# Jarvis73/PEMP

Hardware: AMD Instinct MI355X
Metric: episodes/sec (PEMP stage-1 eval step, PASCAL-5i-shaped 1-shot, ResNet-50) (higher is better)
Workload: dtype f32

## Files before the change

### include/pemp_hip.h

```cpp
#ifndef PEMP_HIP_H
#define PEMP_HIP_H

#include <stddef.h>
#include <stdint.h>

#ifdef __cplusplus
extern "C" {
#endif

#define PEMP_ABI_VERSION 2

#define PEMP_CONV_RELU 1u
#define PEMP_CONV_SHIFT_PER_IMAGE 2u
#define PEMP_CONV_STEM4 4u
#define PEMP_CONV_POOL3S2 8u

typedef struct pemp_conv_desc {
    int32_t N, H, W;
    int32_t Cin, ldx;
    int32_t Ho, Wo;
    int32_t Cout, ldy;
    int32_t KH, KW;
    int32_t stride, pad, dil;
    int32_t ldr;
    int32_t Kpad;
    uint32_t flags;
    int32_t tile;
} pemp_conv_desc;

const char* pemp_last_error(void);
// ... 245 lines not shown
```

### pemp_amd/_lib.py

```python
import ctypes as C
import os

import torch

_HERE = os.path.dirname(os.path.abspath(__file__))
LIB_PATH = os.environ.get("PEMP_HIP_LIB", os.path.join(_HERE, "libpemp_hip.so"))

c_fp = C.c_void_p
c_int = C.c_int
c_size = C.c_size_t


class ConvDesc(C.Structure):
    _fields_ = [(n, C.c_int32) for n in
                ("N", "H", "W", "Cin", "ldx", "Ho", "Wo", "Cout", "ldy", "KH", "KW",
                 "stride", "pad", "dil", "ldr", "Kpad")] + [("flags", C.c_uint32), ("tile", C.c_int32)]


class SampleDesc(C.Structure):
    _fields_ = [("img_off", C.c_int64), ("msk_off", C.c_int64), ("img_out", C.c_int64), ("msk_out", C.c_int64)] + \
               [(n, C.c_int32) for n in ("hs", "ws", "sh", "sw", "oy", "ox", "flip", "jitter_order")] + \
               [("jitter", C.c_float * 3), ("mask_mode", C.c_int32), ("ksx", C.c_int32), ("ksy", C.c_int32),
                ("ws_off", C.c_int64)]


CONV_RELU = 1
CONV_SHIFT_PER_IMAGE = 2
CONV_STEM4 = 4
CONV_POOL3S2 = 8

SYMBOLS = {
    "pemp_last_error": (C.c_char_p, []),
    "pemp_abi_version": (c_int, []),
    "pemp_conv2d_hybrid_rows": (c_int, [C.POINTER(ConvDesc)]),
    "pemp_conv2d_tile_shape": (c_int, [c_int, C.POINTER(c_int), C.POINTER(c_int)]),
    "pemp_conv2d_nhwc_f32": (c_int, [C.POINTER(ConvDesc), c_fp, c_fp, c_fp, c_fp, c_fp, c_fp, c_fp]),
    "pemp_conv2d_padv_splitk_nhwc_f32": (c_int, [C.POINTER(ConvDesc), c_fp, c_fp, c_fp, c_fp, c_fp, c_fp, c_fp, c_fp, c_size, c_fp]),
    "pemp_conv2d_padv_nhwc_f32": (c_int, [C.POINTER(ConvDesc), c_fp, c_fp, c_fp, c_fp, c_fp, c_fp, c_fp, c_fp]),
    "pemp_conv2d_group_nhwc_f32": (c_int, [c_int, C.POINTER(ConvDesc)] + [C.POINTER(c_fp)] * 7 + [c_fp]),
    "pemp_conv2d_bf16_nhwc": (c_int, [C.POINTER(ConvDesc), c_fp, c_fp, c_fp, c_fp, c_fp, c_fp, c_fp, c_int, c_fp]),
    "pemp_pack_split3_bf16": (c_int, [c_fp, c_fp, c_int, c_int, c_fp]),
    "pemp_convert_f32_bf16": (c_int, [c_fp, c_fp, C.c_longlong, c_fp]),
    "pemp_convert_bf16_f32": (c_int, [c_fp, c_fp, C.c_longlong, c_fp]),
    "pemp_conv2d_dropblock_nhwc_f32": (c_int, [C.POINTER(ConvDesc), c_fp, c_fp, c_fp, c_fp, c_fp, c_fp, c_fp, c_fp, c_fp, c_size, c_fp]),
# ... 129 lines not shown
```

### pemp_amd/csrc/conv_common.h

```cpp
#pragma once
#include "common.h"

namespace pemp {

typedef __attribute__((ext_vector_type(16))) float f32x16;
typedef __attribute__((ext_vector_type(4))) float v4f;
typedef __attribute__((ext_vector_type(8))) __bf16 bf16x8;
typedef __attribute__((ext_vector_type(2))) unsigned int u32x2;

#define PEMP_CONV_BF16_IO 0x100u

__device__ __forceinline__ v4f load_quad(const float* base, size_t off, unsigned bf16) {
    if (!bf16) return *(const v4f*)(base + off);
    const u32x2 r = *(const u32x2*)((const unsigned short*)base + off);
    return v4f{__builtin_bit_cast(float, r.x << 16), __builtin_bit_cast(float, r.x & 0xFFFF0000u),
               __builtin_bit_cast(float, r.y << 16), __builtin_bit_cast(float, r.y & 0xFFFF0000u)};
}

__device__ __forceinline__ unsigned int bf16_bits(float f) {
    const unsigned int u = __builtin_bit_cast(unsigned int, f);
    if ((u & 0x7FFFFFFFu) > 0x7F800000u) return (u >> 16) | 0x40u;
    return (u + 0x7FFFu + ((u >> 16) & 1u)) >> 16;
}

// ... 32 lines not shown
    float* stats;
    const uint32_t* bmask;
    const float* bz;
    const float* bmean;
    const float* binvstd;
    int ldbz;
    const float* rowmask;
    const int* rowcnt;
    float* sk_ws;
    int* sk_cnt;
    int sk_full, sk_S;
    int N, H, W, Cin, ldx, Ho, Wo, Cout, ldy, KH, KW, stride, pad, dil, ldr, Kpad;
    unsigned flags;
    int M, HoWo, cin_steps, nk, ntaps;
    int bm_first = 0;
};

constexpr int CONV_GROUP_MAX = 4;
struct ConvGroupArgs {
    ConvArgs a[CONV_GROUP_MAX];
    int first[CONV_GROUP_MAX + 1];
    int nblk[CONV_GROUP_MAX];
    int n;
};

__device__ __forceinline__ int xcd_tile_order(int bid, int nblk) {
    const int x = bid & 7, idx = bid >> 3;
    const int q = nblk >> 3, rem = nblk & 7;
    return (x < rem ? x * (q + 1) : rem * (q + 1) + (x - rem) * q) + idx;
}
// ... 192 lines not shown
```

### pemp_amd/csrc/conv_dma2.hip

```cpp
#include "conv_tiles.h"

#ifndef PEMP_SK_ACQUIRE
#define PEMP_SK_ACQUIRE 1
#endif

namespace pemp {

typedef __attribute__((address_space(3))) void* lptr_t;

template <int BM, int BN, int WGM, int NW, bool PADV, int EPI = 0, bool SK = false, bool BF16 = false, bool DB = false, bool R16 = false,
          bool S3 = false>
__device__ __forceinline__ void conv_dma2_body(const ConvArgs& a, const int bid, const int nblk) {
#if defined(__HIP_DEVICE_COMPILE__)
    constexpr int WGN = NW / WGM;
    constexpr int RPI = NW * 8;
    constexpr int WM = BM / WGM, WN = BN / WGN;
    static_assert(!R16 || (WM == 16 && WN % 16 == 0 && EPI == 0 && !SK && !BF16 && !DB), "R16: 16-row wave tiles, plain epilogue only");
    static_assert(!S3 || (EPI == 0 && !BF16 && !DB && !R16), "S3: plain epilogue, fp32 operands");
    constexpr int TM = R16 ? 1 : WM / 32, TN = R16 ? WN / 16 : WN / 32;
    constexpr int BQ = S3 ? 12 : 8;
    static_assert(!S3 || (BN * BQ) % (NW * 64) == 0, "S3: whole B DMA rounds");
    constexpr int AL = BM / RPI, BL = S3 ? BN * BQ / (NW * 64) : BN / RPI;
    constexpr int NMF = S3 ? 6 * TM * TN : R16 ? 2 * TN : TM * TN * (BF16 ? 1 : 4), NDS = S3 ? 2 * TM + 3 * TN : R16 ? 1 + TN : TM + TN,
                  NDMA = AL + BL;
// ... 27 lines not shown
    } else {
        tile_id = xcd_tile_order(bid, nblk);
    }
    const int bm = a.bm_first + tile_id / ntn;
    const int bn = tile_id % ntn;
    const int m0 = bm * BM, n0 = bn * BN;

    const int p = tid & 7;
    const int r = tid >> 3;
    const int sq = p ^ ((r >> 1) & 7);

    const int bias_pix = a.pad * a.W + a.pad;
    const __amdgpu_buffer_rsrc_t rx =
        __builtin_amdgcn_make_buffer_rsrc((void*)(a.x - (ptrdiff_t)bias_pix * a.ldx), 0, 0x80000000u, 0x00020000);
    const __amdgpu_buffer_rsrc_t rw = __builtin_amdgcn_make_buffer_rsrc((void*)a.w, 0, 0x80000000u, 0x00020000);

    const unsigned padv_off = PADV ? (unsigned)((const char*)a.padv - (const char*)(a.x - (ptrdiff_t)bias_pix * a.ldx)) + sq * 16 : 0x80000000u;
    unsigned a_voff[AL], a_inv[AL], b_voff[BL];
#pragma unroll
    for (int i = 0; i < AL; ++i) {
        const int m = m0 + r + RPI * i;
        const bool ok = m < a.M;
        const int mm = ok ? m : 0;
        const int img = mm / a.HoWo;
        const int rem = mm - img * a.HoWo;
        const int ho = rem / a.Wo;
        const int wo = rem - ho * a.Wo;
        const int hi0 = ho * a.stride - a.pad;
        const int wi0 = wo * a.stride - a.pad;
        a_voff[i] = (unsigned)(((img * a.H + hi0) * a.W + wi0 + bias_pix) * a.ldx + sq * 4) * 4u;
// ... 32 lines not shown
            kw_i = __builtin_amdgcn_readfirstlane(tap0 - kh0 * a.KW);
        }
    }
    const int tapw = a.dil * a.ldx * 4, taph = a.dil * a.W * a.ldx * 4;

#define PEMP_DMA2(buf_)                                                                                           \
    do {                                                                                                          \
        v4f* Ad_ = As + (buf_) * BM * 8 + wave * 64;                                                              \
        v4f* Bd_ = Bs + (buf_) * BN * BQ + wave * 64;                                                             \
        const int sa_ = kh_i * taph + kw_i * tapw + cb * 128;                                                     \
        const int sb_ = (tap * a.Cin + cb * 32) * (S3 ? 6 : 4);                                                   \
        const int sh_ = 31 - tap;                                                                                 \
        const unsigned oob_ = PADV ? padv_off - (unsigned)(kh_i * taph + kw_i * tapw) : 0x80000000u;              \
        _Pragma("unroll") for (int i = 0; i < AL; ++i) {                                                          \
            const unsigned vo_ = ((int)(a_inv[i] << sh_) < 0) ? oob_ : a_voff[i];                                 \
            __builtin_amdgcn_raw_ptr_buffer_load_lds(rx, (lptr_t)(Ad_ + i * RPI * 8), 16, vo_, sa_, 0, 0);        \
        }                                                                                                         \
        _Pragma("unroll") for (int i = 0; i < BL; ++i)                                                            \
            __builtin_amdgcn_raw_ptr_buffer_load_lds(rw, (lptr_t)(Bd_ + i * RPI * 8), 16, b_voff[i], sb_, 0, 0);  \
    } while (0)

    int multi, s_kw, s_ntaps;
    asm volatile("s_nop 0\n\tv_readfirstlane_b32 %0, %3\n\tv_readfirstlane_b32 %1, %4\n\tv_readfirstlane_b32 %2, %5\n\ts_nop 4"
                 : "=s"(multi), "=s"(s_kw), "=s"(s_ntaps)
                 : "v"(a.ntaps > 1 ? 1 : 0), "v"(a.KW), "v"(a.ntaps));
#define PEMP_ADVANCE2()                                                                                           \
    do {                                                                                                          \
        int wt_;                                                                                                  \
        asm volatile(                                                                                             \
            "s_add_u32 %0, %0, %5\n\t"                                      \
            "s_add_u32 %2, %2, %5\n\t"                                      \
            "s_cmp_eq_u32 %2, %6\n\t"                                       \
            "s_cselect_b32 %2, 0, %2\n\t"                                   \
            "s_addc_u32 %1, %1, 0\n\t"                                      \
            "s_xor_b32 %4, %5, 1\n\t"                                       \
            "s_cmp_eq_u32 %0, %7\n\t"                                       \
            "s_cselect_b32 %4, 1, %4\n\t"                                                                          \
            "s_cmp_lg_u32 %4, 0\n\t"                                                                               \
            "s_cselect_b32 %0, 0, %0\n\t"                             \
            "s_cselect_b32 %1, 0, %1\n\t"                                                                          \
            "s_cselect_b32 %2, 0, %2\n\t"                                                                          \
            "s_addc_u32 %3, %3, 0"                                                                                \
            : "+s"(tap), "+s"(kh_i), "+s"(kw_i), "+s"(cb), "=&s"(wt_)                                             \
            : "s"(multi), "s"(s_kw), "s"(s_ntaps)                                                    \
            : "scc");                                                                                             \
    } while (0)

    f32x16 acc[R16 ? 1 : TM][R16 ? 1 : TN];
#pragma unroll
    for (int mi = 0; mi < (R16 ? 1 : TM); ++mi)
#pragma unroll
        for (int ni = 0; ni < (R16 ? 1 : TN); ++ni)
#pragma unroll
            for (int e = 0; e < 16; ++e) acc[mi][ni][e] = 0.f;
    v4f acc16[R16 ? TN : 1];
#pragma unroll
    for (int ni = 0; ni < (R16 ? TN : 1); ++ni) acc16[ni] = v4f{0.f, 0.f, 0.f, 0.f};

    PEMP_DMA2(0);
    if (nkl > 1) {
        PEMP_ADVANCE2();
// ... 117 lines not shown
        if (DMA_) {                         \
            _Pragma("unroll") for (int k_ = 0; k_ < NMF; ++k_) {                                                  \
                __builtin_amdgcn_sched_group_barrier(0x008, 1, 0);                                                \
                _Pragma("unroll") for (int q_ = 0; q_ < PER; ++q_) {                                              \
                    const int it_ = k_ * PER + q_;                                                                \
                    if (it_ < NDS) __builtin_amdgcn_sched_group_barrier(0x100, 1, 0);                             \
                    else if (it_ < NDS + NDMA) __builtin_amdgcn_sched_group_barrier(0x020, 1, 0);                 \
                }                                                                                                 \
            }                                                                                                     \
        }                                                                                                         \
        __builtin_amdgcn_sched_barrier(0);                                                                        \
    } while (0)

    int kt = 0;
    PEMP_READ(0, 0, 0);
    for (; kt + 2 < nkl; ++kt) {
        const int buf = kt & 1;
        PEMP_STEP(buf, true, true);
    }
    if (kt + 1 < nkl) {
        const int buf = kt & 1;
        PEMP_STEP(buf, false, true);
        ++kt;
    }
    constexpr bool PRE = !R16 && TM * TN <= 2;
    v4f rpre[PRE ? TM * TN * 4 : 1];
#pragma unroll
    for (int i = 0; i < (PRE ? TM * TN * 4 : 1); ++i) rpre[i] = v4f{0.f, 0.f, 0.f, 0.f};
    if constexpr (PRE) {
        if (a.res) {
            const int rr_ = lane >> 3, c4_ = (lane & 7) * 4;
#pragma unroll
            for (int mi = 0; mi < TM; ++mi)
#pragma unroll
// ... 150 lines not shown
                        o.y = fmaxf(o.y, 0.f);
                        o.z = fmaxf(o.z, 0.f);
                        o.w = fmaxf(o.w, 0.f);
                    }
                    store_quad(a.y, (size_t)m * a.ldy + n, o, a.flags & PEMP_CONV_BF16_IO);
                }
            }
            asm volatile("s_waitcnt lgkmcnt(0)" ::: "memory");
        }
    }
}

template <int BM, int BN, int WGM, int NW, bool PADV>
__device__ __forceinline__ void conv_dma2_s3p_body(const ConvArgs& a) {
#if defined(__HIP_DEVICE_COMPILE__)
    constexpr bool S3 = true, R16 = false, BF16 = false;
    constexpr int WGN = NW / WGM;
    constexpr int RPI = NW * 8;
    constexpr int WM = BM / WGM, WN = BN / WGN;
    constexpr int TM = WM / 32, TN = WN / 32;
    constexpr int BQ = 12;
    static_assert((BN * BQ) % (NW * 64) == 0, "S3: whole B DMA rounds");
    constexpr int AL = BM / RPI, BL = BN * BQ / (NW * 64);
    constexpr int NMF = 6 * TM * TN, NDS = 2 * TM + 3 * TN, NDMA = AL + BL;
    constexpr int PER = (NDS + NDMA + NMF - 1) / NMF;
    constexpr int NST = TM * TN * 4;
    static_assert(NDMA + NST <= 63, "vmcnt range");
    static_assert(NW <= BM / 32 + 3 * BN / 64, "one 4 KB transpose patch per wave inside ONE stage buffer");

    extern __shared__ __attribute__((aligned(16))) v4f smem[];
    v4f* As = smem;
// ... 12 lines not shown
    const int q8 = T >> 3, r8 = T & 7;
    const int t_first = xcd < r8 ? xcd * (q8 + 1) : r8 * (q8 + 1) + (xcd - r8) * q8;
    const int t_cnt = q8 + (xcd < r8 ? 1 : 0);
    const int gx = ((int)gridDim.x - xcd + 7) >> 3;
    if (idx >= t_cnt) return;
    int j = idx;
    int m0 = (a.bm_first + (t_first + j) / ntn) * BM, n0 = ((t_first + j) % ntn) * BN;

    const int p = tid & 7;
    const int r = tid >> 3;
    const int sq = p ^ ((r >> 1) & 7);
    const int bias_pix = a.pad * a.W + a.pad;
    const __amdgpu_buffer_rsrc_t rx =
        __builtin_amdgcn_make_buffer_rsrc((void*)(a.x - (ptrdiff_t)bias_pix * a.ldx), 0, 0x80000000u, 0x00020000);
    const __amdgpu_buffer_rsrc_t rw = __builtin_amdgcn_make_buffer_rsrc((void*)a.w, 0, 0x80000000u, 0x00020000);
    const unsigned padv_off = PADV ? (unsigned)((const char*)a.padv - (const char*)(a.x - (ptrdiff_t)bias_pix * a.ldx)) + sq * 16 : 0x80000000u;
    unsigned a_voff[AL], a_inv[AL], b_voff[BL];
    auto offsets = [&](const int m0_, const int n0_) {
#pragma unroll
        for (int i = 0; i < AL; ++i) {
            const int m = m0_ + r + RPI * i;
            const bool ok = m < a.M;
            const int mm = ok ? m : 0;
            const int img = mm / a.HoWo;
            const int rem = mm - img * a.HoWo;
            const int ho = rem / a.Wo;
            const int wo = rem - ho * a.Wo;
            const int hi0 = ho * a.stride - a.pad;
            const int wi0 = wo * a.stride - a.pad;
            a_voff[i] = (unsigned)(((img * a.H + hi0) * a.W + wi0 + bias_pix) * a.ldx + sq * 4) * 4u;
// ... 52 lines not shown
    int pb = 0;
    for (;;) {
        f32x16 acc[TM][TN];
#pragma unroll
        for (int mi = 0; mi < TM; ++mi)
#pragma unroll
            for (int ni = 0; ni < TN; ++ni)
#pragma unroll
                for (int e = 0; e < 16; ++e) acc[mi][ni][e] = 0.f;
        const int jn = j + gx;
        const bool more = jn < t_cnt;
        const int m0n = more ? (a.bm_first + (t_first + jn) / ntn) * BM : m0, n0n = more ? ((t_first + jn) % ntn) * BN : n0;

        int kt = 0;
        PEMP_READ(0, pb, 0);
        for (; kt + 2 < nkl; ++kt) {
            const int buf = (kt + pb) & 1;
            PEMP_STEP(buf, true, true);
        }
        if (more) {
            offsets(m0n, n0n);
        } else {
#pragma unroll
            for (int i = 0; i < AL; ++i) {
                a_voff[i] = 0x80000000u;
                a_inv[i] = 0u;
            }
#pragma unroll
            for (int i = 0; i < BL; ++i) b_voff[i] = 0x80000000u;
        }
        tap = 0;
        cb = 0;
        kh_i = 0;
        kw_i = 0;
        if (kt + 1 < nkl) {
            const int buf = (kt + pb) & 1;
            PEMP_STEP_X(buf, true, true, false, true);
            ++kt;
        }
        const int bl = (kt + pb) & 1;
        v4f rres[TM * TN * 4], scv[TN], shv[TN];
        auto epi_loads = [&]() {
            const bool per_img = a.flags & PEMP_CONV_SHIFT_PER_IMAGE;
#pragma unroll
            for (int ni = 0; ni < TN; ++ni) {
                const int n = n0 + wn0 + ni * 32 + c4_;
                scv[ni] = a.scale ? *(const v4f*)(a.scale + n) : v4f{1.f, 1.f, 1.f, 1.f};
                shv[ni] = (a.shift && !per_img) ? *(const v4f*)(a.shift + n) : v4f{0.f, 0.f, 0.f, 0.f};
            }
// ... 39 lines not shown
        m0 = m0n;
        n0 = n0n;
        pb = pbn;
    }
#endif
}

template <int BM, int BN, int WGM, int NW, bool PADV>
__global__ __launch_bounds__(NW * 64) __attribute__((amdgpu_waves_per_eu(BM == 64 ? 4 : 2))) void conv_dma2_s3p_kernel(ConvArgs a) {
    conv_dma2_s3p_body<BM, BN, WGM, NW, PADV>(a);
}
#undef PEMP_STEP_X
#undef PEMP_STEP
#undef PEMP_DMA2
#undef PEMP_ADVANCE2
#undef PEMP_READ
#undef PEMP_MMA

template <int BM, int BN, int WGM, int NW, bool PADV, bool R16 = false, bool S3 = false>
__global__ __launch_bounds__(NW * 64) void conv_dma2_group_kernel(ConvGroupArgs g) {
    int which = 0;
#pragma unroll
    for (int i = 1; i < CONV_GROUP_MAX; ++i) which += (i < g.n && (int)blockIdx.x >= g.first[i]) ? 1 : 0;
    const int bid = (int)blockIdx.x - g.first[which];
    if (bid >= g.nblk[which]) return;
    conv_dma2_body<BM, BN, WGM, NW, PADV, 0, false, false, false, R16, S3>(g.a[which], bid, g.nblk[which]);
}


template <class T, bool PADV, int EPI = 0, bool SK = false, bool BF16 = false, bool DB = false, bool R16 = false, bool S3 = false>
// ... 124 lines not shown
    if (grid < 0) return -1;
    return with_tile<FamSplitK>(shape, [&](auto t) {
        using T = decltype(t);
        return launch_with_lds(dma2_fp32_kernel<T, true>(a), grid, T::NW * 64, tile_lds<T>(), st, a, "conv_dma2/splitk");
    });
}

static int split3_check(bool shape_ok, int shape, const ConvArgs& a) {
    if (shape_ok && !a.stats && !a.rowmask && !(a.flags & PEMP_CONV_BF16_IO)) return 0;
    set_error("conv split3: tile %d / epilogue outside the family", shape);
    return -1;
}

int launch_conv_dma2_split3(int shape, ConvArgs a, void* ws, size_t ws_bytes, bool split, hipStream_t st) {
    if (split3_check(in_family<FamSplit3>(shape), shape, a)) return -1;
    const SplitKPlan p = split ? conv_dma2_splitk_plan(shape, a) : SplitKPlan{0, 0, 1, 0};
    const int sk_grid = p.pieces >= 2 ? bind_splitk(a, p, ws, ws_bytes) : 0;
    if (sk_grid < 0) return -1;
    return with_tile<FamSplit3>(shape, [&](auto t) {
        using T = decltype(t);
        auto kern = sk_grid ? (a.padv ? dma2_kernel<T, true, 0, true, false, false, false, true> : dma2_kernel<T, false, 0, true, false, false, false, true>)
                            : (a.padv ? dma2_kernel<T, true, 0, false, false, false, false, true> : dma2_kernel<T, false, 0, false, false, false, false, true>);
        return launch_with_lds(kern, sk_grid ? sk_grid : tile_grid<T>(a), T::NW * 64, tile_lds_s3<T>(), st, a,
                               sk_grid ? "conv_dma2/split3/splitk" : "conv_dma2/split3");
    });
}

template <class T>
static int launch_dma2_s3p(const ConvArgs& a, hipStream_t st) {
    constexpr size_t lds = tile_lds_s3<T>();
// ... 87 lines not shown
```

### pemp_amd/csrc/conv_igemm.hip

```cpp
#include "conv_tiles.h"

namespace pemp {


template <int BM, int BN, int WGM, bool STEM>
__global__ __launch_bounds__(256) void conv_igemm_kernel(ConvArgs a) {
    constexpr int WGN = 4 / WGM;
    constexpr int WM = BM / WGM, WN = BN / WGN;
    constexpr int TM = WM / 32, TN = WN / 32;
    constexpr int AL = BM / 32, BL = BN / 32;
    static_assert(TM >= 1 && TN >= 1, "wave tile");

    extern __shared__ __attribute__((aligned(16))) v4f smem[];
    v4f* As = smem;
    v4f* Bs = smem + 2 * 8 * BM;

    const int tid = threadIdx.x;
    const int lane = tid & 63;
    const int wave = tid >> 6;
    const int wm0 = (wave / WGN) * WM;
    const int wn0 = (wave % WGN) * WN;
    const int lr = lane & 31, lh = lane >> 5;

    const int ntn = a.Cout / BN;
// ... 202 lines not shown

extern "C" int pemp_conv2d_splitk_nhwc_f32(const pemp_conv_desc* d, const float* x, const float* w, float* y,
                                           const float* scale, const float* shift, const float* residual, void* ws,
                                           size_t ws_bytes, void* stream) {
    return conv2d_impl(d, x, w, y, scale, shift, residual, nullptr, ws, ws_bytes, stream);
}

extern "C" int pemp_conv2d_padv_splitk_nhwc_f32(const pemp_conv_desc* d, const float* x, const float* w, float* y,
                                                const float* scale, const float* shift, const float* residual,
                                                const float* pad_value, void* ws, size_t ws_bytes, void* stream) {
    PEMP_REQUIRE(pad_value, "conv2d_padv_splitk: pad_value is null");
    return conv2d_impl(d, x, w, y, scale, shift, residual, pad_value, ws, ws_bytes, stream);
}

static int conv_fill(const pemp_conv_desc* d, const float* x, const float* w, float* y, const float* scale, const float* shift,
                     const float* residual, const float* pad_value, ConvArgs& a, bool any_taps = false, bool pooled = false) {
    PEMP_REQUIRE(d && x && w && y, "conv2d: null pointer");
    PEMP_REQUIRE(pooled || !(d->flags & PEMP_CONV_POOL3S2), "conv2d: PEMP_CONV_POOL3S2 belongs to pemp_conv2d_nhwc_f32 (no grouped / dropblock / statistics / bf16 form)");
    PEMP_REQUIRE(!pad_value || (!(d->flags & PEMP_CONV_STEM4) && (any_taps || d->KH * d->KW > 1) && ((uintptr_t)pad_value & 15) == 0),
                 "conv2d: pad_value needs a multi-tap non-stem conv and a 16-byte aligned [Cin] vector");
    PEMP_REQUIRE(d->N > 0 && d->H > 0 && d->W > 0 && d->Cin > 0 && d->Cout > 0, "conv2d: bad dims");
    PEMP_REQUIRE(d->KH > 0 && d->KW > 0 && d->stride > 0 && d->dil > 0 && d->pad >= 0, "conv2d: bad kernel geometry");
    const int ho = (d->H + 2 * d->pad - d->dil * (d->KH - 1) - 1) / d->stride + 1;
    const int wo = (d->W + 2 * d->pad - d->dil * (d->KW - 1) - 1) / d->stride + 1;
    PEMP_REQUIRE(ho == d->Ho && wo == d->Wo, "conv2d: Ho/Wo (%d,%d) do not match geometry (%d,%d)", d->Ho, d->Wo, ho, wo);
    PEMP_REQUIRE(d->Cout % 64 == 0, "conv2d: Cout=%d must be a multiple of 64", d->Cout);
    PEMP_REQUIRE(d->ldy >= d->Cout && d->ldy % 4 == 0 && ((uintptr_t)y & 15) == 0, "conv2d: ldy must be >= Cout and a multiple of 4, y 16-byte aligned");
    PEMP_REQUIRE(!scale || ((uintptr_t)scale & 15) == 0, "conv2d: scale must be 16-byte aligned");
    PEMP_REQUIRE(!shift || ((uintptr_t)shift & 15) == 0, "conv2d: shift must be 16-byte aligned");
    PEMP_REQUIRE(((uintptr_t)x & 15) == 0 && ((uintptr_t)w & 15) == 0, "conv2d: x/w must be 16-byte aligned");
    const bool stem = d->flags & PEMP_CONV_STEM4;
    const int ntaps = d->KH * d->KW;
    if (stem) {
        PEMP_REQUIRE(d->Cin == 4 && d->ldx == 4, "conv2d: STEM4 needs NHWC4 input (Cin=ldx=4)");
        PEMP_REQUIRE(d->Kpad % 32 == 0 && d->Kpad >= ntaps * 4, "conv2d: STEM4 Kpad=%d too small / not x32", d->Kpad);
    } else {
        PEMP_REQUIRE(d->Cin % 32 == 0, "conv2d: Cin=%d must be a multiple of 32 (or use STEM4)", d->Cin);
        PEMP_REQUIRE(d->ldx >= d->Cin && d->ldx % 4 == 0, "conv2d: ldx=%d must be >= Cin and a multiple of 4", d->ldx);
        PEMP_REQUIRE(d->Kpad == ntaps * d->Cin, "conv2d: Kpad=%d must equal KH*KW*Cin=%d", d->Kpad, ntaps * d->Cin);
    }
    const long long in_elems = (long long)d->N * d->H * d->W * d->ldx;
    const long long out_elems = (long long)d->N * d->Ho * d->Wo * (long long)(d->ldy > d->ldr ? d->ldy : d->ldr);
    PEMP_REQUIRE(in_elems < (1ll << 31) && out_elems < (1ll << 31), "conv2d: tensor too large for 32-bit indexing");

    a.x = x; a.w = w; a.y = y; a.scale = scale; a.shift = shift; a.res = residual; a.padv = pad_value; a.stats = nullptr; a.bz = nullptr;
    a.bmask = nullptr; a.bmean = nullptr; a.binvstd = nullptr; a.ldbz = 0;
    a.rowmask = nullptr; a.rowcnt = nullptr;
    a.N = d->N; a.H = d->H; a.W = d->W; a.Cin = d->Cin; a.ldx = d->ldx; a.Ho = d->Ho; a.Wo = d->Wo;
    a.Cout = d->Cout; a.ldy = d->ldy; a.KH = d->KH; a.KW = d->KW; a.stride = d->stride; a.pad = d->pad;
    a.dil = d->dil; a.ldr = d->ldr; a.Kpad = d->Kpad; a.flags = d->flags;
    a.HoWo = d->Ho * d->Wo;
    a.M = d->N * a.HoWo;
    a.ntaps = ntaps;
    a.cin_steps = stem ? 1 : d->Cin / 32;
    a.nk = d->Kpad / 32;
    if (residual) PEMP_REQUIRE(d->ldr >= d->Cout && d->ldr % 4 == 0 && ((uintptr_t)residual & 15) == 0, "conv2d: ldr must be >= Cout and x4, residual 16-byte aligned");
    a.sk_ws = nullptr; a.sk_cnt = nullptr; a.sk_full = 0; a.sk_S = 1;
    a.bm_first = 0;
    return 0;
}

static int conv2d_impl(const pemp_conv_desc* d, const float* x, const float* w, float* y, const float* scale, const float* shift,
                       const float* residual, const float* pad_value, void* ws, size_t ws_bytes, void* stream) {
    ConvArgs a;
    const int rc = conv_fill(d, x, w, y, scale, shift, residual, pad_value, a, false, true);
    if (rc) return rc;
    const bool stem = d->flags & PEMP_CONV_STEM4;
    int tile = d->tile;
    if (tile == 0) {
        tile = 3;
    }
    TileId t = decode_tile(tile);
    if (d->flags & PEMP_CONV_POOL3S2) {
        PEMP_REQUIRE(stem && t.family == TILE_SPLIT3 && !t.splitk && !residual && !pad_value,
                     "conv2d: PEMP_CONV_POOL3S2 needs PEMP_CONV_STEM4 with split3 weights (a tile id 41..49), no residual, no padding value");
        return launch_conv_stem_pool(a, (hipStream_t)stream);
    }
    PEMP_REQUIRE(tile != 33 && tile != 53, "conv2d: no split-K variant of the 64 x 64 tile");
    PEMP_REQUIRE(tile != 45 && tile != 55, "conv2d: no split3 form of the 128 x 64 8-wave tile");
    PEMP_REQUIRE(tile != 48, "conv2d: no persistent split3 form of the 128 x 128 4-wave tile");
    PEMP_REQUIRE(t.exists, "conv2d: unknown tile id %d", tile);
    hipStream_t st = (hipStream_t)stream;
    if (t.family == TILE_SPLIT3) {
        PEMP_REQUIRE(!stem && conv_dma2_supported(a) && (long long)a.Cout * a.Kpad * 6 < (1ll << 31),
                     "conv2d: split3 tile %d needs a geometry of the buffer-addressed kernels (no stem, <= 32 taps, operands < 2 GiB)", tile);
        PEMP_REQUIRE_COUT("conv2d", t.shape, a.Cout);
        if (t.persistent) return launch_conv_dma2_split3_persist(t.shape, a, st);
        return launch_conv_dma2_split3(t.shape, a, ws, ws_bytes, t.splitk, st);
    }
    if (t.family == TILE_DMA2 && t.splitk) {
        if (conv_dma2_supported(a)) {
            PEMP_REQUIRE_COUT("conv2d", t.shape, a.Cout);
// ... 111 lines not shown
    h.Kpad = d->Kpad / 2;
    ConvArgs a;
    const int rc = conv_fill(&h, (const float*)x, (const float*)w, (float*)y, scale, shift, (const float*)residual,
                             (const float*)pad_value, a);
    if (rc) return rc;
    if (!out_f32) a.flags |= PEMP_CONV_BF16_IO;
    PEMP_REQUIRE(conv_dma2_supported(a), "conv2d_bf16: geometry / operand size outside the buffer-addressed kernels");
    PEMP_REQUIRE_COUT("conv2d_bf16", t.shape, a.Cout);
    return launch_conv_dma2_bf16(t.shape, a, (hipStream_t)stream);
}


static TileId stats_tile(const pemp_conv_desc* d) { return decode_tile(d->tile == 0 ? 23 : d->tile); }

static int conv_stats_fill(const char* what, const pemp_conv_desc* d, ConvArgs& a) {
    PEMP_REQUIRE(!(d->flags & (PEMP_CONV_STEM4 | PEMP_CONV_RELU | PEMP_CONV_SHIFT_PER_IMAGE | PEMP_CONV_POOL3S2)), "%s: plain conv only (no stem / ReLU / per-image shift)", what);
    PEMP_REQUIRE(d->N > 0 && d->H > 0 && d->W > 0 && d->Cin > 0 && d->Cout > 0 && d->KH > 0 && d->KW > 0 && d->stride > 0 && d->dil > 0 && d->pad >= 0,
                 "%s: bad geometry", what);
    const int ho = (d->H + 2 * d->pad - d->dil * (d->KH - 1) - 1) / d->stride + 1;
    const int wo = (d->W + 2 * d->pad - d->dil * (d->KW - 1) - 1) / d->stride + 1;
    PEMP_REQUIRE(ho == d->Ho && wo == d->Wo, "%s: Ho/Wo do not match geometry", what);
    PEMP_REQUIRE(d->Cout % 64 == 0 && d->Cin % 32 == 0 && d->ldx >= d->Cin && d->ldx % 4 == 0 && d->ldy >= d->Cout && d->ldy % 4 == 0,
                 "%s: Cout %% 64, Cin %% 32, strides %% 4", what);
    PEMP_REQUIRE(d->Kpad == d->KH * d->KW * d->Cin, "%s: Kpad must equal KH*KW*Cin", what);
    a.scale = nullptr; a.shift = nullptr; a.padv = nullptr; a.rowmask = nullptr; a.rowcnt = nullptr;
    a.N = d->N; a.H = d->H; a.W = d->W; a.Cin = d->Cin; a.ldx = d->ldx; a.Ho = d->Ho; a.Wo = d->Wo;
    a.Cout = d->Cout; a.ldy = d->ldy; a.KH = d->KH; a.KW = d->KW; a.stride = d->stride; a.pad = d->pad;
    a.dil = d->dil; a.ldr = d->ldr; a.Kpad = d->Kpad; a.flags = d->flags;
    a.HoWo = d->Ho * d->Wo;
    a.M = d->N * a.HoWo;
    a.ntaps = d->KH * d->KW;
// ... 74 lines not shown
```

### pemp_amd/engine.py

```python
import os

import torch
import torch.nn as nn

from . import ops
from .ops import ConvParams

BN_EPS = 1e-5

SPLIT3 = os.environ.get("PEMP_SPLIT3", "1") != "0"


def with_split3(cp):
    if not SPLIT3 or cp.w.dtype != torch.float32:
        return cp
    if cp.stem:
        if (cp.kh, cp.kw, cp.stride, cp.pad, cp.dil) == (7, 7, 2, 3, 1) and cp.kpad == 224 and cp.cout % 64 == 0:
            cp.w3pool = ops.pack_split3(cp.w)
    elif cp.kh * cp.kw <= 32 and cp.cin % 32 == 0 and cp.cout % 64 == 0 and cp.kpad == cp.kh * cp.kw * cp.cin:
        cp.w3 = ops.pack_split3(cp.w)
    return cp


def bn_affine(bn):
    invstd = 1.0 / torch.sqrt(bn.running_var.detach().float() + bn.eps)
# ... 29 lines not shown
        self.dtype = dtype
        self.bufs = {}
        self.ws = {}

    def get(self, name, shape, dtype=None, zero=False):
        dtype = self.dtype if dtype is None else dtype
        key = (name, tuple(shape), dtype)
        t = self.bufs.get(key)
        if t is None:
            t = (torch.zeros if zero else torch.empty)(shape, dtype=dtype, device=self.device)
            self.bufs[key] = t
        return t


class _BlockPlan:
    def __init__(self, blk, extra_in=0, dtype=torch.float32):
        sl = None
        if extra_in:
            sl = (0, blk.conv1.weight.shape[1] - extra_in)
        self.c1 = conv_params(blk.conv1, blk.bn1, relu=True, in_slice=sl, dtype=dtype)
        self.c2 = conv_params(blk.conv2, blk.bn2, relu=True, dtype=dtype)
        self.c3 = conv_params(blk.conv3, blk.bn3, relu=True, dtype=dtype)
        self.ds = conv_params(blk.downsample[0], blk.downsample[1], relu=False, in_slice=sl, dtype=dtype) \
            if blk.downsample is not None else None
        if extra_in:
            self.c1_extra = (blk.conv1.weight.detach()[:, sl[1]:, 0, 0].float() * self.c1.scale[:, None]).contiguous()
            self.ds_extra = (blk.downsample[0].weight.detach()[:, sl[1]:, 0, 0].float() * self.ds.scale[:, None]).contiguous()


class ResNetEngine:

    def __init__(self, prm, arena):
        self.arena = arena
        self.stem = conv_params(prm.conv1, prm.bn1, relu=True, stem4=True)
        self.stages = []
        for name in ("layer1", "layer2", "layer3"):
            self.stages.append([_BlockPlan(b, dtype=arena.dtype) for b in getattr(prm, name)])

    def _block(self, x, bp, tag, c1_shift=None, ds_shift=None, out=None):
        a = self.arena
        n, h, w, _ = x.shape
        ho = ops.conv_out_size(h, 1, bp.c1.stride, 0, 1)
        wo = ops.conv_out_size(w, 1, bp.c1.stride, 0, 1)
        if out is None:
            out = a.get(("blk", tag), (n, ho, wo, bp.c3.cout))
        if bp.ds is not None and c1_shift is None and ds_shift is None and 0 < n * ho * wo <= GROUP_MAX_ROWS and x.dtype == torch.float32:
            y1, res = ops.conv2d_group([x, x], [bp.c1, bp.ds], [a.get("y1", (n, ho, wo, bp.c1.cout)),
                                                                a.get("res", (n, ho, wo, bp.ds.cout))])
            y2 = ops.conv2d(y1, bp.c2, out=a.get("y2", (n, ho, wo, bp.c2.cout)))
            return ops.conv2d(y2, bp.c3, out=out, residual=res)
        y1 = ops.conv2d(x, bp.c1, out=a.get("y1", (n, ho, wo, bp.c1.cout)),
                        shift_override=c1_shift, per_image_shift=c1_shift is not None)
        y2 = ops.conv2d(y1, bp.c2, out=a.get("y2", (n, ho, wo, bp.c2.cout)))
        if bp.ds is not None:
            res = ops.conv2d(x, bp.ds, out=a.get("res", (n, ho, wo, bp.ds.cout)),
                             shift_override=ds_shift, per_image_shift=ds_shift is not None)
        else:
            res = x
        return ops.conv2d(y2, bp.c3, out=out, residual=res)

# ... 247 lines not shown
```

### pemp_amd/ops.py

```python
import ctypes as C
import collections
import json
import os

import torch

from . import _lib
from ._lib import ConvDesc, CONV_RELU, CONV_SHIFT_PER_IMAGE, CONV_STEM4, CONV_POOL3S2


def _stream():
    return C.c_void_p(torch.cuda.current_stream().cuda_stream)


def _p(t):
    return C.c_void_p(t.data_ptr()) if t is not None else C.c_void_p(0)


def _chk_dev(*ts):
    for t in ts:
        if t is not None and (not t.is_cuda):
            raise _lib.PempHipError("pemp_amd ops need device (cuda/HIP) tensors; there is no CPU path")


# ... 7 lines not shown
        ld = t.stride(1)
    elif n > 1:
        ld = t.stride(0)
    else:
        ld = c
    if (w > 1 and h > 1 and t.stride(1) != w * ld) or (h * w > 1 and n > 1 and t.stride(0) != h * w * ld):
        raise ValueError(f"{name}: pixels must be densely packed with stride ld={ld}, got strides {t.stride()}")
    return ld


def conv_out_size(i, k, s, p, d):
    return (i + 2 * p - d * (k - 1) - 1) // s + 1


class ConvParams:
    __slots__ = ("w", "scale", "shift", "cin", "cout", "kh", "kw", "stride", "pad", "dil", "kpad", "stem", "relu", "w3", "w3pool")

    def __init__(self, w, scale, shift, cin, cout, kh, kw, stride, pad, dil, kpad, stem, relu, w3=None, w3pool=None):
        self.w, self.scale, self.shift, self.w3, self.w3pool = w, scale, shift, w3, w3pool
        self.cin, self.cout, self.kh, self.kw = cin, cout, kh, kw
        self.stride, self.pad, self.dil, self.kpad, self.stem, self.relu = stride, pad, dil, kpad, stem, relu


_SHAPES = {1: (128, 128), 2: (128, 64), 3: (64, 64), 4: (128, 128), 5: (128, 64), 6: (256, 128), 7: (256, 256),
           8: (32, 64),
           9: (64, 64)}
Tile = collections.namedtuple("Tile", "shape family splitk persistent_of")
SPLIT3_PERSISTENT = {47: 43, 49: 46}
TILES = {base + s: Tile(_SHAPES[s], family, base in (30, 50), None)
         for family, base, shapes in (("igemm", 0, (1, 2, 3)),
                                      ("dma", 10, range(1, 8)),
                                      ("dma2", 20, range(1, 10)),
                                      ("dma2", 30, (1, 2, 4, 5, 6, 7)),
# ... 273 lines not shown
        raise ValueError(f"stem_pool: fp32 NHWC4 input expected, got {cin} channels of {x.dtype}")
    ho, wo = conv_out_size(h, 7, 2, 3, 1), conv_out_size(w, 7, 2, 3, 1)
    hp, wp = _pool_out(ho, 3, 2, 1, True), _pool_out(wo, 3, 2, 1, True)
    if out is None:
        out = torch.empty((n, hp, wp, p.cout), dtype=torch.float32, device=x.device)
    ldy = _nhwc(out, "out")
    if tuple(out.shape) != (n, hp, wp, p.cout) or out.dtype != torch.float32:
        raise ValueError(f"stem_pool: out shape {tuple(out.shape)} != {(n, hp, wp, p.cout)} (fp32)")
    flags = CONV_STEM4 | CONV_POOL3S2 | (CONV_RELU if p.relu else 0)
    d = ConvDesc(n, h, w, cin, ldx, ho, wo, p.cout, ldy, 7, 7, 2, 3, 1, 0, p.kpad, flags, SPLIT3_DEFAULT_TILE)
    _lib.check(lib.pemp_conv2d_nhwc_f32(C.byref(d), _p(x), _p(p.w3pool), _p(out), _p(p.scale), _p(p.shift), None, _stream()),
               "pemp_conv2d_nhwc_f32")
    return out


def _conv2d_bf16(x, p, out, residual, shift_override, per_image_shift, relu, tile, pad_value):
    lib = _lib.load()
    _chk_dev(x, p.w, out, residual, pad_value)
    if p.w.dtype != torch.bfloat16 or p.stem:
        raise ValueError("conv2d (bf16 input): the layer's weights must be packed as bf16 (engine precision 'bf16'); no stem")
    n, h, w, cin, ldx, ho, wo, out, ldy, ldr = _conv_geom("conv2d", x, p, out, residual, torch.bfloat16,
                                                          None if out is None else out.dtype)
    out_f32 = out.dtype == torch.float32
    if pad_value is not None and (pad_value.numel() != cin or pad_value.dtype != torch.bfloat16 or not pad_value.is_contiguous()):
        raise ValueError(f"conv2d: pad_value must be a contiguous bf16 [{cin}] vector")
    shift = p.shift if shift_override is None else shift_override
    flags = (CONV_RELU if (p.relu if relu is None else relu) else 0) | (CONV_SHIFT_PER_IMAGE if per_image_shift else 0)

    def launch(t):
        d = ConvDesc(n, h, w, cin, ldx, ho, wo, p.cout, ldy, p.kh, p.kw, p.stride, p.pad, p.dil, ldr, p.kpad, flags, t)
# ... 649 lines not shown
```

Before: 1339.

## Fuse bottleneck downsample 1x1 into conv3 as a dual-source K-concatenated GEMM

For ResNet bottleneck blocks that have a downsample branch, the conv3 1x1 and downsample 1x1 convolutions are merged into one GEMM. Their BN-folded weights are concatenated along K, and the kernel switches its A-operand buffer resource and offsets partway through the K loop, moving from y2 to the strided block input x. This removes the separate downsample launch and the write and re-read of its residual tensor. In exchange the kernel carries an extra branch and offset recomputation in the split3 K loop, and the fused path gives up split-K.

```diff
diff --git a/include/pemp_hip.h b/include/pemp_hip.h
--- a/include/pemp_hip.h
+++ b/include/pemp_hip.h
@@ -14,6 +14,10 @@
 #define PEMP_CONV_SHIFT_PER_IMAGE 2u
 #define PEMP_CONV_STEM4 4u
 #define PEMP_CONV_POOL3S2 8u
+
+#define PEMP_CONV_DUAL1X1 16u
+#define PEMP_CONV_DUAL_K1_SHIFT 16
+#define PEMP_CONV_DUAL_K1(steps) ((uint32_t)(steps) << PEMP_CONV_DUAL_K1_SHIFT)
 
 typedef struct pemp_conv_desc {
     int32_t N, H, W;
diff --git a/pemp_amd/_lib.py b/pemp_amd/_lib.py
--- a/pemp_amd/_lib.py
+++ b/pemp_amd/_lib.py
@@ -28,6 +28,8 @@
 CONV_SHIFT_PER_IMAGE = 2
 CONV_STEM4 = 4
 CONV_POOL3S2 = 8
+CONV_DUAL1X1 = 16
+CONV_DUAL_K1_SHIFT = 16
 
 SYMBOLS = {
     "pemp_last_error": (C.c_char_p, []),
diff --git a/pemp_amd/csrc/conv_common.h b/pemp_amd/csrc/conv_common.h
--- a/pemp_amd/csrc/conv_common.h
+++ b/pemp_amd/csrc/conv_common.h
@@ -70,6 +70,8 @@
     unsigned flags;
     int M, HoWo, cin_steps, nk, ntaps;
     int bm_first = 0;
+    const float* x2 = nullptr;
+    int nk1 = 0, H2 = 0, W2 = 0, stride2 = 0, ldx2 = 0;
 };
 
 constexpr int CONV_GROUP_MAX = 4;
diff --git a/pemp_amd/csrc/conv_dma2.hip b/pemp_amd/csrc/conv_dma2.hip
--- a/pemp_amd/csrc/conv_dma2.hip
+++ b/pemp_amd/csrc/conv_dma2.hip
@@ -65,6 +65,7 @@
     const __amdgpu_buffer_rsrc_t rx =
         __builtin_amdgcn_make_buffer_rsrc((void*)(a.x - (ptrdiff_t)bias_pix * a.ldx), 0, 0x80000000u, 0x00020000);
     const __amdgpu_buffer_rsrc_t rw = __builtin_amdgcn_make_buffer_rsrc((void*)a.w, 0, 0x80000000u, 0x00020000);
+    __amdgpu_buffer_rsrc_t rxc = rx;
 
     const unsigned padv_off = PADV ? (unsigned)((const char*)a.padv - (const char*)(a.x - (ptrdiff_t)bias_pix * a.ldx)) + sq * 16 : 0x80000000u;
     unsigned a_voff[AL], a_inv[AL], b_voff[BL];
@@ -127,7 +128,7 @@
         const unsigned oob_ = PADV ? padv_off - (unsigned)(kh_i * taph + kw_i * tapw) : 0x80000000u;              \
         _Pragma("unroll") for (int i = 0; i < AL; ++i) {                                                          \
             const unsigned vo_ = ((int)(a_inv[i] << sh_) < 0) ? oob_ : a_voff[i];                                 \
-            __builtin_amdgcn_raw_ptr_buffer_load_lds(rx, (lptr_t)(Ad_ + i * RPI * 8), 16, vo_, sa_, 0, 0);        \
+            __builtin_amdgcn_raw_ptr_buffer_load_lds(rxc, (lptr_t)(Ad_ + i * RPI * 8), 16, vo_, sa_, 0, 0);        \
         }                                                                                                         \
         _Pragma("unroll") for (int i = 0; i < BL; ++i)                                                            \
             __builtin_amdgcn_raw_ptr_buffer_load_lds(rw, (lptr_t)(Bd_ + i * RPI * 8), 16, b_voff[i], sb_, 0, 0);  \
@@ -158,6 +159,34 @@
             : "s"(multi), "s"(s_kw), "s"(s_ntaps)                                                    \
             : "scc");                                                                                             \
     } while (0)
+
+#define PEMP_SWITCH2(m0_)                                                                                         \
+    do {                                                                                                          \
+        _Pragma("unroll") for (int i = 0; i < AL; ++i) {                                                          \
+            const int m = (m0_) + r + RPI * i;                                                                    \
+            const int mm = m < a.M ? m : 0;                                                                       \
+            const int img = mm / a.HoWo;                                                                          \
+            const int rem = mm - img * a.HoWo;                                                                    \
+            const int ho = rem / a.Wo;                                                                            \
+            const int wo = rem - ho * a.Wo;                                                                       \
+            a_voff[i] = (unsigned)(((img * a.H2 + ho * a.stride2) * a.W2 + wo * a.stride2) * a.ldx2 + sq * 4) * 4u; \
+        }                                                                                                         \
+        _Pragma("unroll") for (int i = 0; i < BL; ++i) b_voff[i] += (unsigned)a.nk1 * 192u;                       \
+        cb = -1;                                                                                                  \
+        rxc = __builtin_amdgcn_make_buffer_rsrc((void*)a.x2, 0, 0x80000000u, 0x00020000);                         \
+    } while (0)
+#define PEMP_KLOOP(buf_of_kt_, m0_)                                                                               \
+    do {                                                                                                          \
+        const int ksw_ = (S3 && !SK_ && a.nk1) ? a.nk1 - 2 : -1;                                                  \
+        for (; kt + 2 < nkl; ++kt) {                                                                              \
+            if constexpr (S3 && !SK_) {                                                                           \
+                if (kt == ksw_) PEMP_SWITCH2(m0_);                                                                \
+            }                                                                                                     \
+            const int buf = (buf_of_kt_) & 1;                                                                     \
+            PEMP_STEP(buf, true, true);                                                                           \
+        }                                                                                                         \
+    } while (0)
+    constexpr bool SK_ = SK;
 
     f32x16 acc[R16 ? 1 : TM][R16 ? 1 : TN];
 #pragma unroll
@@ -305,10 +334,7 @@
 
     int kt = 0;
     PEMP_READ(0, 0, 0);
-    for (; kt + 2 < nkl; ++kt) {
-        const int buf = kt & 1;
-        PEMP_STEP(buf, true, true);
-    }
+    PEMP_KLOOP(kt, m0);
     if (kt + 1 < nkl) {
         const int buf = kt & 1;
         PEMP_STEP(buf, false, true);
@@ -489,7 +515,7 @@
 template <int BM, int BN, int WGM, int NW, bool PADV>
 __device__ __forceinline__ void conv_dma2_s3p_body(const ConvArgs& a) {
 #if defined(__HIP_DEVICE_COMPILE__)
-    constexpr bool S3 = true, R16 = false, BF16 = false;
+    constexpr bool S3 = true, R16 = false, BF16 = false, SK_ = false;
     constexpr int WGN = NW / WGM;
     constexpr int RPI = NW * 8;
     constexpr int WM = BM / WGM, WN = BN / WGN;
@@ -532,6 +558,7 @@
     const __amdgpu_buffer_rsrc_t rx =
         __builtin_amdgcn_make_buffer_rsrc((void*)(a.x - (ptrdiff_t)bias_pix * a.ldx), 0, 0x80000000u, 0x00020000);
     const __amdgpu_buffer_rsrc_t rw = __builtin_amdgcn_make_buffer_rsrc((void*)a.w, 0, 0x80000000u, 0x00020000);
+    __amdgpu_buffer_rsrc_t rxc = rx;
     const unsigned padv_off = PADV ? (unsigned)((const char*)a.padv - (const char*)(a.x - (ptrdiff_t)bias_pix * a.ldx)) + sq * 16 : 0x80000000u;
     unsigned a_voff[AL], a_inv[AL], b_voff[BL];
     auto offsets = [&](const int m0_, const int n0_) {
@@ -614,10 +641,7 @@
 
         int kt = 0;
         PEMP_READ(0, pb, 0);
-        for (; kt + 2 < nkl; ++kt) {
-            const int buf = (kt + pb) & 1;
-            PEMP_STEP(buf, true, true);
-        }
+        PEMP_KLOOP(kt + pb, m0);
         if (more) {
             offsets(m0n, n0n);
         } else {
@@ -633,6 +657,7 @@
         cb = 0;
         kh_i = 0;
         kw_i = 0;
+        rxc = rx;
         if (kt + 1 < nkl) {
             const int buf = (kt + pb) & 1;
             PEMP_STEP_X(buf, true, true, false, true);
@@ -702,6 +727,8 @@
 #undef PEMP_STEP
 #undef PEMP_DMA2
 #undef PEMP_ADVANCE2
+#undef PEMP_SWITCH2
+#undef PEMP_KLOOP
 #undef PEMP_READ
 #undef PEMP_MMA
 
@@ -856,6 +883,10 @@
 
 int launch_conv_dma2_split3(int shape, ConvArgs a, void* ws, size_t ws_bytes, bool split, hipStream_t st) {
     if (split3_check(in_family<FamSplit3>(shape), shape, a)) return -1;
+    if (a.nk1 && split) {
+        set_error("conv split3: the dual-source 1x1 has no split-K form");
+        return -1;
+    }
     const SplitKPlan p = split ? conv_dma2_splitk_plan(shape, a) : SplitKPlan{0, 0, 1, 0};
     const int sk_grid = p.pieces >= 2 ? bind_splitk(a, p, ws, ws_bytes) : 0;
     if (sk_grid < 0) return -1;
diff --git a/pemp_amd/csrc/conv_igemm.hip b/pemp_amd/csrc/conv_igemm.hip
--- a/pemp_amd/csrc/conv_igemm.hip
+++ b/pemp_amd/csrc/conv_igemm.hip
@@ -240,9 +240,10 @@
 }
 
 static int conv_fill(const pemp_conv_desc* d, const float* x, const float* w, float* y, const float* scale, const float* shift,
-                     const float* residual, const float* pad_value, ConvArgs& a, bool any_taps = false, bool pooled = false) {
+                     const float* residual, const float* pad_value, ConvArgs& a, bool any_taps = false, bool plain_entry = false) {
     PEMP_REQUIRE(d && x && w && y, "conv2d: null pointer");
-    PEMP_REQUIRE(pooled || !(d->flags & PEMP_CONV_POOL3S2), "conv2d: PEMP_CONV_POOL3S2 belongs to pemp_conv2d_nhwc_f32 (no grouped / dropblock / statistics / bf16 form)");
+    PEMP_REQUIRE(plain_entry || !(d->flags & PEMP_CONV_POOL3S2), "conv2d: PEMP_CONV_POOL3S2 belongs to pemp_conv2d_nhwc_f32 (no grouped / dropblock / statistics / bf16 form)");
+    PEMP_REQUIRE(plain_entry || !(d->flags & PEMP_CONV_DUAL1X1), "conv2d: PEMP_CONV_DUAL1X1 belongs to pemp_conv2d_nhwc_f32 (no grouped / dropblock / statistics / bf16 form)");
     PEMP_REQUIRE(!pad_value || (!(d->flags & PEMP_CONV_STEM4) && (any_taps || d->KH * d->KW > 1) && ((uintptr_t)pad_value & 15) == 0),
                  "conv2d: pad_value needs a multi-tap non-stem conv and a 16-byte aligned [Cin] vector");
     PEMP_REQUIRE(d->N > 0 && d->H > 0 && d->W > 0 && d->Cin > 0 && d->Cout > 0, "conv2d: bad dims");
@@ -262,7 +263,8 @@
         PEMP_REQUIRE(d->Kpad % 32 == 0 && d->Kpad >= ntaps * 4, "conv2d: STEM4 Kpad=%d too small / not x32", d->Kpad);
     } else {
         PEMP_REQUIRE(d->Cin % 32 == 0, "conv2d: Cin=%d must be a multiple of 32 (or use STEM4)", d->Cin);
-        PEMP_REQUIRE(d->ldx >= d->Cin && d->ldx % 4 == 0, "conv2d: ldx=%d must be >= Cin and a multiple of 4", d->ldx);
+        const int cin_x = (d->flags & PEMP_CONV_DUAL1X1) ? 4 : d->Cin;
+        PEMP_REQUIRE(d->ldx >= cin_x && d->ldx % 4 == 0, "conv2d: ldx=%d must be >= %d and a multiple of 4", d->ldx, cin_x);
         PEMP_REQUIRE(d->Kpad == ntaps * d->Cin, "conv2d: Kpad=%d must equal KH*KW*Cin=%d", d->Kpad, ntaps * d->Cin);
     }
     const long long in_elems = (long long)d->N * d->H * d->W * d->ldx;
@@ -280,9 +282,21 @@
     a.ntaps = ntaps;
     a.cin_steps = stem ? 1 : d->Cin / 32;
     a.nk = d->Kpad / 32;
-    if (residual) PEMP_REQUIRE(d->ldr >= d->Cout && d->ldr % 4 == 0 && ((uintptr_t)residual & 15) == 0, "conv2d: ldr must be >= Cout and x4, residual 16-byte aligned");
+    if (residual && (d->flags & PEMP_CONV_DUAL1X1)) PEMP_REQUIRE(d->ldr % 4 == 0 && ((uintptr_t)residual & 15) == 0, "conv2d: PEMP_CONV_DUAL1X1 ldr must be a multiple of 4, the first source 16-byte aligned");
+    else if (residual) PEMP_REQUIRE(d->ldr >= d->Cout && d->ldr % 4 == 0 && ((uintptr_t)residual & 15) == 0, "conv2d: ldr must be >= Cout and x4, residual 16-byte aligned");
     a.sk_ws = nullptr; a.sk_cnt = nullptr; a.sk_full = 0; a.sk_S = 1;
     a.bm_first = 0;
+    a.x2 = nullptr; a.nk1 = 0; a.H2 = a.W2 = a.stride2 = a.ldx2 = 0;
+    if (d->flags & PEMP_CONV_DUAL1X1) {
+        const int nk1 = (int)(d->flags >> PEMP_CONV_DUAL_K1_SHIFT), c1 = nk1 * 32, c2 = d->Cin - c1;
+        PEMP_REQUIRE(residual && !pad_value && !stem, "conv2d: PEMP_CONV_DUAL1X1 takes its first source in the residual slot; no padding value, no stem");
+        PEMP_REQUIRE(d->KH == 1 && d->KW == 1 && d->pad == 0, "conv2d: PEMP_CONV_DUAL1X1 is a 1x1 conv without padding");
+        PEMP_REQUIRE(nk1 >= 2 && c2 >= 32, "conv2d: PEMP_CONV_DUAL1X1 needs >= 64 channels of the first source (flags bits 16..31: its 32-channel K steps) and >= 32 of the second, Cin = their sum (got %d of %d)", c1, d->Cin);
+        PEMP_REQUIRE(d->ldr >= c1 && d->ldx >= c2, "conv2d: PEMP_CONV_DUAL1X1 per-pixel strides %d / %d below the sources' channels %d / %d", d->ldr, d->ldx, c1, c2);
+        a.x2 = x; a.H2 = d->H; a.W2 = d->W; a.stride2 = d->stride; a.ldx2 = d->ldx; a.nk1 = nk1;
+        a.x = residual; a.H = d->Ho; a.W = d->Wo; a.stride = 1; a.ldx = d->ldr; a.res = nullptr;
+        a.flags = d->flags & ((1u << PEMP_CONV_DUAL_K1_SHIFT) - 1u);
+    }
     return 0;
 }
 
@@ -302,6 +316,8 @@
                      "conv2d: PEMP_CONV_POOL3S2 needs PEMP_CONV_STEM4 with split3 weights (a tile id 41..49), no residual, no padding value");
         return launch_conv_stem_pool(a, (hipStream_t)stream);
     }
+    PEMP_REQUIRE(!a.nk1 || (t.family == TILE_SPLIT3 && !t.splitk), "conv2d: PEMP_CONV_DUAL1X1 needs a split3 tile id 41..49 (no split-K form)");
+    PEMP_REQUIRE(!a.nk1 || (long long)a.N * a.H2 * a.W2 * a.ldx2 * 4 < (1ll << 31), "conv2d: PEMP_CONV_DUAL1X1 second source of 2 GiB or more");
     PEMP_REQUIRE(tile != 33 && tile != 53, "conv2d: no split-K variant of the 64 x 64 tile");
     PEMP_REQUIRE(tile != 45 && tile != 55, "conv2d: no split3 form of the 128 x 64 8-wave tile");
     PEMP_REQUIRE(tile != 48, "conv2d: no persistent split3 form of the 128 x 128 4-wave tile");
@@ -443,7 +459,7 @@
 static TileId stats_tile(const pemp_conv_desc* d) { return decode_tile(d->tile == 0 ? 23 : d->tile); }
 
 static int conv_stats_fill(const char* what, const pemp_conv_desc* d, ConvArgs& a) {
-    PEMP_REQUIRE(!(d->flags & (PEMP_CONV_STEM4 | PEMP_CONV_RELU | PEMP_CONV_SHIFT_PER_IMAGE | PEMP_CONV_POOL3S2)), "%s: plain conv only (no stem / ReLU / per-image shift)", what);
+    PEMP_REQUIRE(!(d->flags & (PEMP_CONV_STEM4 | PEMP_CONV_RELU | PEMP_CONV_SHIFT_PER_IMAGE | PEMP_CONV_POOL3S2 | PEMP_CONV_DUAL1X1)), "%s: plain conv only (no stem / ReLU / per-image shift / dual source)", what);
     PEMP_REQUIRE(d->N > 0 && d->H > 0 && d->W > 0 && d->Cin > 0 && d->Cout > 0 && d->KH > 0 && d->KW > 0 && d->stride > 0 && d->dil > 0 && d->pad >= 0,
                  "%s: bad geometry", what);
     const int ho = (d->H + 2 * d->pad - d->dil * (d->KH - 1) - 1) / d->stride + 1;
diff --git a/pemp_amd/engine.py b/pemp_amd/engine.py
--- a/pemp_amd/engine.py
+++ b/pemp_amd/engine.py
@@ -9,6 +9,8 @@
 BN_EPS = 1e-5
 
 SPLIT3 = os.environ.get("PEMP_SPLIT3", "1") != "0"
+FUSE_DS = os.environ.get("PEMP_FUSE_DS", "1") != "0"
+FUSE_DS_STAGES = frozenset(os.environ.get("PEMP_FUSE_DS_STAGES", "layer1,layer2,layer3").split(","))
 
 
 def with_split3(cp):
@@ -68,7 +70,7 @@
 
 
 class _BlockPlan:
-    def __init__(self, blk, extra_in=0, dtype=torch.float32):
+    def __init__(self, blk, extra_in=0, dtype=torch.float32, fuse_ds=False):
         sl = None
         if extra_in:
             sl = (0, blk.conv1.weight.shape[1] - extra_in)
@@ -80,6 +82,9 @@
         if extra_in:
             self.c1_extra = (blk.conv1.weight.detach()[:, sl[1]:, 0, 0].float() * self.c1.scale[:, None]).contiguous()
             self.ds_extra = (blk.downsample[0].weight.detach()[:, sl[1]:, 0, 0].float() * self.ds.scale[:, None]).contiguous()
+        self.fused = False
+        if fuse_ds and FUSE_DS and self.ds is not None and not extra_in and self.c3.w3 is not None and self.ds.w3 is not None:
+            self.fused = ops.fuse_downsample(self.c3, self.ds)
 
 
 class ResNetEngine:
@@ -89,7 +94,7 @@
         self.stem = conv_params(prm.conv1, prm.bn1, relu=True, stem4=True)
         self.stages = []
         for name in ("layer1", "layer2", "layer3"):
-            self.stages.append([_BlockPlan(b, dtype=arena.dtype) for b in getattr(prm, name)])
+            self.stages.append([_BlockPlan(b, dtype=arena.dtype, fuse_ds=name in FUSE_DS_STAGES) for b in getattr(prm, name)])
 
     def _block(self, x, bp, tag, c1_shift=None, ds_shift=None, out=None):
         a = self.arena
@@ -98,6 +103,10 @@
         wo = ops.conv_out_size(w, 1, bp.c1.stride, 0, 1)
         if out is None:
             out = a.get(("blk", tag), (n, ho, wo, bp.c3.cout))
+        if bp.fused and c1_shift is None and ds_shift is None and x.dtype == torch.float32:
+            y1 = ops.conv2d(x, bp.c1, out=a.get("y1", (n, ho, wo, bp.c1.cout)))
+            y2 = ops.conv2d(y1, bp.c2, out=a.get("y2", (n, ho, wo, bp.c2.cout)))
+            return ops.conv2d_dual(y2, x, bp.c3, bp.ds, out=out)
         if bp.ds is not None and c1_shift is None and ds_shift is None and 0 < n * ho * wo <= GROUP_MAX_ROWS and x.dtype == torch.float32:
             y1, res = ops.conv2d_group([x, x], [bp.c1, bp.ds], [a.get("y1", (n, ho, wo, bp.c1.cout)),
                                                                 a.get("res", (n, ho, wo, bp.ds.cout))])
diff --git a/pemp_amd/ops.py b/pemp_amd/ops.py
--- a/pemp_amd/ops.py
+++ b/pemp_amd/ops.py
@@ -6,7 +6,7 @@
 import torch
 
 from . import _lib
-from ._lib import ConvDesc, CONV_RELU, CONV_SHIFT_PER_IMAGE, CONV_STEM4, CONV_POOL3S2
+from ._lib import ConvDesc, CONV_RELU, CONV_SHIFT_PER_IMAGE, CONV_STEM4, CONV_POOL3S2, CONV_DUAL1X1, CONV_DUAL_K1_SHIFT
 
 
 def _stream():
@@ -45,9 +45,11 @@
 
 
 class ConvParams:
-    __slots__ = ("w", "scale", "shift", "cin", "cout", "kh", "kw", "stride", "pad", "dil", "kpad", "stem", "relu", "w3", "w3pool")
+    __slots__ = ("w", "scale", "shift", "cin", "cout", "kh", "kw", "stride", "pad", "dil", "kpad", "stem", "relu", "w3", "w3pool",
+                 "w3ds", "shift_ds")
 
     def __init__(self, w, scale, shift, cin, cout, kh, kw, stride, pad, dil, kpad, stem, relu, w3=None, w3pool=None):
+        self.w3ds = self.shift_ds = None
         self.w, self.scale, self.shift, self.w3, self.w3pool = w, scale, shift, w3, w3pool
         self.cin, self.cout, self.kh, self.kw = cin, cout, kh, kw
         self.stride, self.pad, self.dil, self.kpad, self.stem, self.relu = stride, pad, dil, kpad, stem, relu
@@ -351,6 +353,62 @@
     return out
 
 
+def fold_dual_weight(c3, ds):
+    if c3.scale is None or ds.scale is None or c3.shift is None or ds.shift is None or c3.cout != ds.cout:
+        return None
+    if (c3.kh, c3.kw, c3.stride, c3.pad, ds.kh, ds.kw, ds.pad) != (1, 1, 1, 0, 1, 1, 0) or c3.stem or ds.stem:
+        return None
+    if c3.w.dtype != torch.float32 or ds.w.dtype != torch.float32:
+        return None
+    s = torch.cat([c3.scale, ds.scale])
+    if not bool(torch.isfinite(s).all()) or bool((s == 0).any()):
+        return None
+    w = torch.cat([c3.w * c3.scale[:, None], ds.w * ds.scale[:, None]], dim=1).contiguous()
+    return w, (c3.shift + ds.shift).contiguous()
+
+
+def fuse_downsample(c3, ds):
+    if c3.cin % 32 or c3.cin < 64 or ds.cin % 32 or c3.cout % 64:
+        return False
+    f = fold_dual_weight(c3, ds)
+    if f is None:
+        return False
+    c3.w3ds, c3.shift_ds = pack_split3(f[0]), f[1]
+    return True
+
+
+def conv2d_dual(y2, x, c3, ds, out=None, relu=None, tile=0):
+    lib = _lib.load()
+    if c3.w3ds is None:
+        raise ValueError("conv2d_dual: the layer carries no dual-source weights (fuse_downsample)")
+    _chk_dev(y2, x, c3.w3ds, out)
+    ldx = _nhwc(x, "x")
+    ld1 = _nhwc(y2, "y2")
+    n, h, w, c2 = x.shape
+    ho, wo = conv_out_size(h, 1, ds.stride, 0, 1), conv_out_size(w, 1, ds.stride, 0, 1)
+    c1, cout = c3.cin, c3.cout
+    if c2 != ds.cin or tuple(y2.shape) != (n, ho, wo, c1):
+        raise ValueError(f"conv2d_dual: x {tuple(x.shape)} / y2 {tuple(y2.shape)} do not match the layers ({ds.cin} channels at stride "
+                         f"{ds.stride}, {c1} channels of {(n, ho, wo)})")
+    if out is None:
+        out = torch.empty((n, ho, wo, cout), dtype=torch.float32, device=x.device)
+    ldy = _nhwc(out, "out")
+    if tuple(out.shape) != (n, ho, wo, cout):
+        raise ValueError(f"conv2d_dual: out shape {tuple(out.shape)} != {(n, ho, wo, cout)}")
+    flags = CONV_DUAL1X1 | ((c1 // 32) << CONV_DUAL_K1_SHIFT) | (CONV_RELU if (c3.relu if relu is None else relu) else 0)
+
+    def launch(t):
+        d = ConvDesc(n, h, w, c1 + c2, ldx, ho, wo, cout, ldy, 1, 1, ds.stride, 0, 1, ld1, c1 + c2, flags, t)
+        _lib.check(lib.pemp_conv2d_nhwc_f32(C.byref(d), _p(x), _p(c3.w3ds), _p(out), None, _p(c3.shift_ds), _p(y2), _stream()),
+                   "pemp_conv2d_nhwc_f32")
+
+    if tile == 0:
+        key = (c1, c2, cout, 1, 1, ds.stride, 0, 1, 0, n, h, w, 0, 0, 3, 2)
+        tile = _choose_tile(key, n * ho * wo, launch, lambda: _fits(list(SPLIT3_TILES), cout), SPLIT3_DEFAULT_TILE)
+    launch(tile)
+    return out
+
+
 def _conv2d_bf16(x, p, out, residual, shift_override, per_image_shift, relu, tile, pad_value):
     lib = _lib.load()
     _chk_dev(x, p.w, out, residual, pad_value)
diff --git a/scratch/conv_pmc_layers.py b/scratch/conv_pmc_layers.py
--- /dev/null
+++ b/scratch/conv_pmc_layers.py
@@ -0,0 +1,21 @@
+import collections
+import csv
+import sys
+
+per_step, steps = int(sys.argv[1]), int(sys.argv[2])
+conv = [{} for _ in range(steps * per_step)]
+for path in sys.argv[3:]:
+    disp = collections.OrderedDict()
+    for r in csv.DictReader(open(path)):
+        if any(k in r["Kernel_Name"] for k in ("conv_dma", "conv_igemm", "conv_stem_pool")):
+            d = disp.setdefault(int(r["Dispatch_Id"]), {"name": r["Kernel_Name"]})
+            d[r["Counter_Name"]] = d.get(r["Counter_Name"], 0.0) + float(r["Counter_Value"])
+    for c, d in zip(conv, [disp[k] for k in sorted(disp)][-steps * per_step:]):
+        c.update(d)
+print(f"conv launches per step {per_step}, steps {steps}")
+print(f"{'pos':>3} {'FETCH MB':>9} {'WRITE MB':>9}  kernel")
+for p in range(per_step):
+    rs = conv[p::per_step]
+    name = rs[-1]["name"].split("(")[0].replace("void pemp::", "").replace("pemp::", "")
+    f, w = (sum(r.get(c, 0.0) for r in rs) / len(rs) / 1024 for c in ("FETCH_SIZE", "WRITE_SIZE"))
+    print(f"{p:>3} {f:9.1f} {w:9.1f}  {name}")
```

Result: no change. 1348, median of 6 (+0.6%).
